# NVIDIAGameWorks/kaolin-wisp

Measured on NVIDIA B200. Metric: rays/sec (fwd+bwd) 1024^2 Lego NeRF HashGrid, higher is better.
Workload: dtype f16(tensor)+f32 accumulate

## Files before the change

### kaolin-wisp_b200/csrc/wb_shade_tc.cu

```cuda
#include "wb_common.cuh"
#include "wb_featx.cuh"
#include "wb_tc.cuh"
#include <math.h>

#define TC_ML 16
constexpr int TC_ROWS = 128;
constexpr int TC_GROUP = 256;
constexpr int TC_BWD_GROUPS = 2;
constexpr int TC_ISSUERS = 2;

struct WbTc {
    int nl_d, nl_c;
    int I[TC_ML], O[TC_ML], Kp[TC_ML], Np[TC_ML];
    int w_off[TC_ML], b_off[TC_ML];
    int has_bias;
    int ones_off;
    int src_w[TC_ML], src_b[TC_ML];
    int blob_bytes;
    int tile_off[TC_ML];
    int dy_off[2];
    int sub_off[2];
    int w_smem_off;
    int smem_bytes;
    int acc_col[TC_ML];
    int work_col[2];
    int tmem_cols;
    int feat_dim, pos_dim, view_dim, pos_mode, pos_freq, view_mode, view_freq;
    int fits2;
};

static int tc_round_up(int v, int m) { return (v + m - 1) / m * m; }

constexpr int TC_B3_GROUPS = 3;
struct TcB3Plan {
    int P, Q, R, E, GB, blob_off, ones_off, smem_bytes;
    int groups;
    int kind[8], acc_col[8], bias_col[8];
    int acc_begin, acc_end;
};

static bool tc_b3_plan(const WbTc& m, TcB3Plan* p)
{
    if (m.nl_d != 2 || m.nl_c != 3) return false;
    int maxw = 0, sumN = 0;
    for (int l = 0; l < 5; ++l) { maxw = max(maxw, max(m.Kp[l], m.Np[l])); sumN += m.Np[l]; }
    if (maxw > 128) return false;
    if (maxw > 64 && maxw != 128) return false;
    if (m.Kp[1] != maxw || m.Kp[3] != maxw || m.Kp[4] != maxw || m.Np[0] != maxw || m.Np[2] != maxw || m.Np[3] != maxw) return false;
    memset(p, 0, sizeof(*p));
    p->groups = (maxw <= 64 && sumN <= 512 - 3 * 64) ? 3 : 1;
    const int wc = p->groups == 3 ? 64 : 128;
    int col = p->groups * wc;
    p->acc_begin = col;
    for (int l = 0; l < 5; ++l) {
        p->kind[l] = p->groups == 3 ? 0 : (m.Kp[l] + 16 < m.Np[l] ? 2 : (m.Kp[l] >= 128 ? 1 : 0));
        p->acc_col[l] = col; col += p->kind[l] == 2 ? m.Kp[l] + 16 : m.Np[l];
        p->bias_col[l] = col; if (p->kind[l] == 1) col += 16;
    }
    p->acc_end = col;
    if (col > 512) return false;
    const int big = (maxw / 8 + 1) * 2048;
    const int small = (max(m.Np[1], m.Np[4]) / 8) * 2048;
    p->P = 0; p->Q = big; p->R = 2 * big; p->E = 3 * big; p->GB = 3 * big + small;
    p->blob_off = p->groups * p->GB;
    p->ones_off = p->blob_off + m.blob_bytes;
    int end = p->ones_off + 2 * 2048;
    const int window = (p->groups - 1) * p->GB + (p->groups == 3 ? p->R : p->E) + 16 * 2048;
    if (end < window) end = window;
    p->smem_bytes = end + 64;
    return p->smem_bytes + 6144 <= 227 * 1024;
}


static int tc_embed_dim(int mode, int freq) { return mode == 0 ? 0 : mode == 1 ? 3 : mode == 2 ? 6 * freq : 3 + 6 * freq; }

int wb_tc_make(const wb_nef_desc* d, bool backward, WbTc* m, bool tmem_a = false)
{
    WB_CHECK_ARG(d->dens_layers >= 1 && d->col_layers >= 1 && d->dens_layers + d->col_layers <= TC_ML, "unsupported decoder depth");
    WB_CHECK_ARG(d->dens_params && d->col_params, "null decoder parameters");
    memset(m, 0, sizeof(*m));
    m->nl_d = d->dens_layers; m->nl_c = d->col_layers;
    m->feat_dim = d->multiscale == 0 ? d->num_lods * d->feature_dim : d->feature_dim;
    m->pos_mode = d->pos_mode; m->pos_freq = d->pos_freq; m->view_mode = d->view_mode; m->view_freq = d->view_freq;
    m->pos_dim = tc_embed_dim(d->pos_mode, d->pos_freq); m->view_dim = tc_embed_dim(d->view_mode, d->view_freq);
    WB_CHECK_ARG(d->dens_dims[0] == m->feat_dim + m->pos_dim, "decoder_density input width != grid features + position embedding");
    const int dout = d->dens_dims[d->dens_layers];
    WB_CHECK_ARG(dout >= 2 && dout <= 16, "tensor-core path: decoder_density output must be 2..16 wide");
    WB_CHECK_ARG(d->col_dims[0] == dout - 1 + m->view_dim, "decoder_color input width != density feats - 1 + view embedding");
    WB_CHECK_ARG(d->col_dims[d->col_layers] == 3, "decoder_color output must be 3 wide");
    const int nl = m->nl_d + m->nl_c;
    int off = 0, srcd = 0, srcc = 0, maxw = 0;
    for (int l = 0; l < nl; ++l) {
        const bool dens = l < m->nl_d;
        const int I = dens ? d->dens_dims[l] : d->col_dims[l - m->nl_d];
        const int O = dens ? d->dens_dims[l + 1] : d->col_dims[l - m->nl_d + 1];
        WB_CHECK_ARG(I >= 1 && I <= 128 && O >= 1 && O <= 128, "tensor-core path: layer widths must be <= 128");
        m->I[l] = I; m->O[l] = O; m->Kp[l] = tc_round_up(I, 16); m->Np[l] = tc_round_up(O, 16);
        m->w_off[l] = off; off += m->Kp[l] * m->Np[l] * 2;
        m->b_off[l] = off; off += m->Np[l] * 32;
        int& src = dens ? srcd : srcc;
        m->src_w[l] = src; src += I * O;
        if (d->has_bias) { m->src_b[l] = src; src += O; } else m->src_b[l] = -1;
        maxw = max(maxw, max(m->Kp[l], m->Np[l]));
    }
    m->blob_bytes = tc_round_up(off, 16);
    m->has_bias = d->has_bias ? 1 : 0;
    int sub_bytes = 0;
    if (backward) {
        for (int l = 0; l < nl; ++l) { m->tile_off[l] = sub_bytes; sub_bytes += (m->Kp[l] / 8 + 1) * 2048; }
    } else {
        for (int l = 0; l < nl; ++l) m->tile_off[l] = 0;
        sub_bytes = (maxw / 8) * 2048;
    }
    const int groups = backward ? TC_BWD_GROUPS : 1;
    m->sub_off[0] = 0; m->sub_off[1] = sub_bytes;
    int p = groups * sub_bytes;
    if (backward) { m->dy_off[0] = p; p += (maxw / 8) * 2048; m->dy_off[1] = p; p += (maxw / 8) * 2048; }
    m->w_smem_off = p; p += m->blob_bytes;
    m->ones_off = p; p += 2 * 2048;
    if (backward) {
        const int need = m->sub_off[groups - 1] + m->tile_off[nl - 1] + 16 * 2048;
        if (p < need) p = need;
    }
    m->smem_bytes = p + 64;
    const bool smem2 = m->smem_bytes + (backward ? 5632 : 3584) <= 227 * 1024;
    int col = 0;
    for (int gi = 0; gi < groups; ++gi) { m->work_col[gi] = col; col += maxw; }
    if (tmem_a && !backward) { m->work_col[1] = col; col += maxw / 2; }
    if (backward) for (int l = 0; l < nl; ++l) { m->acc_col[l] = col; col += m->Np[l]; }
    m->fits2 = (smem2 && col <= 512) ? 1 : 0;
    if (!m->fits2) {
        TcB3Plan plan3;
        WB_CHECK_ARG(backward && tc_b3_plan(*m, &plan3),
                     !smem2 ? (backward ? "tensor-core path: decoder backward does not fit in shared memory (use precision 0)"
                                        : "tensor-core path: decoder does not fit in shared memory (use precision 0)")
                            : "tensor-core path: accumulators do not fit in TMEM (use precision 0)");
        col = 512;
    }
    int alloc = 32; while (alloc < col) alloc <<= 1;
    m->tmem_cols = alloc;
    return WB_OK;
}

static void tc_dfeat_shape(const wb_nef_desc* d, int* planes, int* width)
{
    *width = d->feature_dim;
    *planes = d->multiscale == 0 ? (d->lod_idx < d->num_lods ? d->lod_idx : d->num_lods) : 1;
    if (*planes < 0) *planes = 0;
}
static int64_t tc_align256(int64_t b) { return (b + 255) / 256 * 256; }

int64_t wb_tc_workspace_bytes(const wb_nef_desc* nef, int64_t R, int64_t S, int backward)
{
    WbTc m; if (wb_tc_make(nef, false, &m)) return -1;
    int planes, width; tc_dfeat_shape(nef, &planes, &width);
    int64_t b = tc_align256(R * m.Kp[m.nl_d] * 2);
    if (backward) b += tc_align256((int64_t)planes * S * width * 2);
    return b + 256;
}
int wb_tc_supported(const wb_nef_desc* nef, int backward)
{
    WbTc m; if (wb_tc_make(nef, false, &m)) return 0;
    if (backward && wb_tc_make(nef, true, &m)) return 0;
    return 1;
}
int64_t wb_tc_feat_bytes(const wb_nef_desc* nef, int64_t S)
{
    WbTc m; if (wb_tc_make(nef, true, &m) || wb_tc_make(nef, false, &m)) return -1;
    return (int64_t)m.Kp[0] * 2 * S + 256;
}

__global__ void wb_tc_pack_kernel(WbTc m, const float* __restrict__ dens, const float* __restrict__ col, uint8_t* __restrict__ blob)
{
    const int nl = m.nl_d + m.nl_c;
    for (int l = 0; l < nl; ++l) {
        const float* src = l < m.nl_d ? dens : col;
        const int I = m.I[l], O = m.O[l], Kp = m.Kp[l], Np = m.Np[l];
        __half* w = reinterpret_cast<__half*>(blob + m.w_off[l]);
        for (int e = blockIdx.x * blockDim.x + threadIdx.x; e < Kp * Np; e += gridDim.x * blockDim.x) {
            const int kc = e / (Np * 8), n = (e / 8) % Np, k = kc * 8 + (e & 7);
            w[e] = __float2half_rn((n < O && k < I) ? src[m.src_w[l] + n * I + k] : 0.0f);
        }
        __half* b = reinterpret_cast<__half*>(blob + m.b_off[l]);
        for (int e = blockIdx.x * blockDim.x + threadIdx.x; e < Np * 16; e += gridDim.x * blockDim.x) {
            const int kc = e / (Np * 8), n = (e / 8) % Np, k = kc * 8 + (e & 7);
            b[e] = __float2half_rn((k == 0 && n < O && m.src_b[l] >= 0) ? src[m.src_b[l] + n] : 0.0f);
// ... 708 lines not shown
                            if (dist >= o) { v0[j] += a; v1[j] += b; }
                        }
                    }
                }
                if (tail && valid) {
                    float2* t2 = reinterpret_cast<float2*>(tb);
#pragma unroll
                    for (int j = 0; j < 4; ++j) {
                        const uint32_t i0 = idx[j], i1 = idx[j + 4];
                        const bool nz0 = (v0[j] != 0.0f || v1[j] != 0.0f), nz1 = (v0[j + 4] != 0.0f || v1[j + 4] != 0.0f);
                        if (pair_ok && ((i0 ^ i1) == 1u)) {
                            if (nz0 || nz1) {
                                const float4 val = (i0 & 1u) ? make_float4(v0[j + 4], v1[j + 4], v0[j], v1[j]) : make_float4(v0[j], v1[j], v0[j + 4], v1[j + 4]);
                                atomicAdd(reinterpret_cast<float4*>(t2 + (i0 & ~1u)), val);
                            }
                        } else {
                            if (nz0) atomicAdd(t2 + i0, make_float2(v0[j], v1[j]));
                            if (nz1) atomicAdd(t2 + i1, make_float2(v0[j + 4], v1[j + 4]));
                        }
                    }
                }
            } else {
                for (int f = 0; f < Fr; ++f) {
                    float v[8];
#pragma unroll
                    for (int j = 0; j < 8; ++j) v[j] = gv[f] * cf[j];
                    for (int o = 1; o <= maxd; o <<= 1) {
#pragma unroll
                        for (int j = 0; j < 8; ++j) { const float a = __shfl_up_sync(0xffffffffu, v[j], o); if (dist >= o) v[j] += a; }
                    }
                    if (tail && valid) {
#pragma unroll
                        for (int j = 0; j < 8; ++j) if (v[j] != 0.0f) atomicAdd(tb + (int64_t)idx[j] * Fr + f, v[j]);
                    }
                }
            }
        }
    }
}

__global__ void __launch_bounds__(256)
wb_featx_scatter_kernel(WbGridX gx, TcIn in, const __half* __restrict__ dfeat, int width, const float* __restrict__ scale_p)
{
    const float inv_scale = 1.0f / __ldg(scale_p);
    const int lane = threadIdx.x & 31;
    const int64_t nwork = (in.S + 31) & ~(int64_t)31;
    for (int64_t s = (int64_t)blockIdx.x * blockDim.x + threadIdx.x; s < nwork; s += (int64_t)gridDim.x * blockDim.x) {
        const bool valid = s < in.S;
        float px = 0.0f, py = 0.0f, pz = 0.0f;
        if (valid) {
            const int64_t ray = __ldg(in.rec_ray + s);
            const float t = __ldg(in.rec_t + s);
            px = wb_addcmul(__ldg(in.origins + 3 * ray), __ldg(in.dirs + 3 * ray), t);
            py = wb_addcmul(__ldg(in.origins + 3 * ray + 1), __ldg(in.dirs + 3 * ray + 1), t);
            pz = wb_addcmul(__ldg(in.origins + 3 * ray + 2), __ldg(in.dirs + 3 * ray + 2), t);
        }
        auto grad = [&](int f) {
            return __half2float(dfeat[((int64_t)(f / width) * in.S + s) * width + (f % width)]) * inv_scale;
        };
        if (gx.kind != 1 || gx.C > 4) {
            if (valid) wb_featx_scatter(gx, px, py, pz, grad);
            continue;
        }
        const int C = gx.C;
        float gsum[3][4];
#pragma unroll
        for (int p = 0; p < 3; ++p)
#pragma unroll
            for (int c = 0; c < 4; ++c) gsum[p][c] = (gx.sum && valid && c < C) ? grad(p * C + c) : 0.0f;
        for (int l = 0; l < gx.nl; ++l) {
            const int size = gx.res[l] + 1; const int64_t hw = (int64_t)size * size;
#pragma unroll
            for (int p = 0; p < 3; ++p) {
                WbBilinear b = wb_tp_setup(px, py, pz, p, size);
                float v[4][4];
#pragma unroll
                for (int c = 0; c < 4; ++c) {
                    const float g = gx.sum ? gsum[p][c] : ((valid && c < C) ? grad((l * 3 + p) * C + c) : 0.0f);
                    v[0][c] = g * b.nw; v[1][c] = g * b.ne; v[2][c] = g * b.sw; v[3][c] = g * b.se;
                }
                const int key = valid ? b.o00 : -1 - lane;
                const int kprev = __shfl_up_sync(0xffffffffu, key, 1);
                const bool head = (lane == 0) || (kprev != key);
                const uint32_t heads = __ballot_sync(0xffffffffu, head);
                const int run_head = 31 - __clz(heads & (0xffffffffu >> (31 - lane)));
                const int dist = lane - run_head;
                const bool tail = (lane == 31) || ((heads >> (lane + 1)) & 1u);
                const int maxd = __reduce_max_sync(0xffffffffu, dist);
                for (int o = 1; o <= maxd; o <<= 1) {
#pragma unroll
                    for (int t4 = 0; t4 < 4; ++t4)
#pragma unroll
                        for (int c = 0; c < 4; ++c) {
                            const float a = __shfl_up_sync(0xffffffffu, v[t4][c], o);
                            if (dist >= o) v[t4][c] += a;
                        }
                }
                if (tail && valid && gx.chlast) {
                    float4* t4 = reinterpret_cast<float4*>(gx.gptr[l * 3 + p]);
                    auto nz = [](const float* q) { return q[0] != 0.0f || q[1] != 0.0f || q[2] != 0.0f || q[3] != 0.0f; };
                    if (nz(v[0])) atomicAdd(t4 + b.o00, make_float4(v[0][0], v[0][1], v[0][2], v[0][3]));
                    if (b.bx1 && nz(v[1])) atomicAdd(t4 + b.o01, make_float4(v[1][0], v[1][1], v[1][2], v[1][3]));
                    if (b.by1 && nz(v[2])) atomicAdd(t4 + b.o10, make_float4(v[2][0], v[2][1], v[2][2], v[2][3]));
                    if (b.bx1 && b.by1 && nz(v[3])) atomicAdd(t4 + b.o11, make_float4(v[3][0], v[3][1], v[3][2], v[3][3]));
                } else if (tail && valid) {
                    float* pl = gx.gptr[l * 3 + p];
#pragma unroll
                    for (int c = 0; c < 4; ++c) {
                        if (c >= C) break;
                        float* ch = pl + c * hw;
                        if (v[0][c] != 0.0f) atomicAdd(ch + b.o00, v[0][c]);
                        if (b.bx1 && v[1][c] != 0.0f) atomicAdd(ch + b.o01, v[1][c]);
                        if (b.by1 && v[2][c] != 0.0f) atomicAdd(ch + b.o10, v[2][c]);
                        if (b.bx1 && b.by1 && v[3][c] != 0.0f) atomicAdd(ch + b.o11, v[3][c]);
                    }
                }
            }
        }
    }
}

#include "wb_shade_tc_bwd3.cuh"

int wb_tc_decoder_bwd_ex(const wb_nef_desc* nef, const float* blob, const wb_rays* rays, const float* rec_t, const int32_t* rec_ray,
                         int64_t S, const float* g_shaded, const float* scale, const void* feat_saved, void* workspace,
                         float* grad_dens, float* grad_col, float* grad_table, int* fused_out, cudaStream_t st);
int wb_tc_decoder_bwd(const wb_nef_desc* nef, const float* blob, const wb_rays* rays, const float* rec_t, const int32_t* rec_ray,
                      int64_t S, const float* g_shaded, const float* scale, const void* feat_saved, void* workspace,
                      float* grad_dens, float* grad_col, cudaStream_t st)
{
    return wb_tc_decoder_bwd_ex(nef, blob, rays, rec_t, rec_ray, S, g_shaded, scale, feat_saved, workspace, grad_dens, grad_col, nullptr, nullptr, st);
}
int wb_tc_decoder_bwd_ex(const wb_nef_desc* nef, const float* blob, const wb_rays* rays, const float* rec_t, const int32_t* rec_ray,
                         int64_t S, const float* g_shaded, const float* scale, const void* feat_saved, void* workspace,
                         float* grad_dens, float* grad_col, float* grad_table, int* fused_out, cudaStream_t st)
{
    if (fused_out) *fused_out = 0;
    WbTc m; int rc = wb_tc_make(nef, true, &m); if (rc) return rc;
    WB_CHECK_ARG(scale != nullptr, "precision 1 needs the device loss-scale pointer");
    WB_CHECK_ARG(feat_saved != nullptr && workspace != nullptr, "precision 1 backward needs the saved features and the workspace");
    if (g_tc_skip_embed) g_tc_skip_embed = 0;
    else { rc = tc_launch_ray_embed(m, rays, workspace, st); if (rc) return rc; }
    int planes, width; tc_dfeat_shape(nef, &planes, &width);
    const int64_t R = rays->num_rays;
    __half* dfeat = reinterpret_cast<__half*>(reinterpret_cast<uint8_t*>(workspace) + tc_align256(R * m.Kp[m.nl_d] * 2));
    TcIn in = { rays->origins, rays->dirs, rec_t, rec_ray, S, reinterpret_cast<const uint4*>(workspace), nullptr, reinterpret_cast<const uint4*>(feat_saved),
                g_tc_s_begin, g_tc_s_end };
    const int64_t S_launch = (g_tc_s_end ? g_tc_s_end : S) - g_tc_s_begin;
    TcGrads G = { grad_dens, grad_col, scale, dfeat, planes, width };
    TcB3Plan plan;
    if (tc_b3_plan(m, &plan)) {
        WbGrid g; memset(&g, 0, sizeof(g));
        const bool fuse = grad_table != nullptr && nef->grid_kind == 0 && nef->feature_dim == 2 && nef->multiscale == 0 && planes <= 16 &&
                          plan.groups == 3;
        if (fuse) { rc = wb_make_grid(nef, &g); if (rc) return rc; }
        using Bwd3Kernel = decltype(&wb_mlp_bwd3_tc_kernel<false, 3>);
        static const Bwd3Kernel kerns3[3] = { wb_mlp_bwd3_tc_kernel<false, 1>, wb_mlp_bwd3_tc_kernel<false, 3>, wb_mlp_bwd3_tc_kernel<true, 3> };
        const int variant = plan.groups == 1 ? 0 : fuse ? 2 : 1;
        const Bwd3Kernel kern3 = kerns3[variant];
        static int64_t done3[3] = { -1, -1, -1 };
        if (done3[variant] != WB_ATTR_KEY(plan.smem_bytes)) {
            WB_CUDA(cudaFuncSetAttribute(kern3, cudaFuncAttributeMaxDynamicSharedMemorySize, plan.smem_bytes));
            done3[variant] = WB_ATTR_KEY(plan.smem_bytes);
        }
        const int64_t nctas3 = ((S_launch + TC_ROWS - 1) / TC_ROWS + plan.groups - 1) / plan.groups;
        int64_t grid3 = (int64_t)wb_num_sms(); if (grid3 > nctas3) grid3 = nctas3;
        kern3<<<(unsigned)grid3, plan.groups * TC_GROUP, plan.smem_bytes, st>>>(m, plan, reinterpret_cast<const uint8_t*>(blob), in,
                                                                          reinterpret_cast<const float4*>(g_shaded), G, g, grad_table);
        WB_LAUNCH_CHECK();
        if (fuse && fused_out) *fused_out = 1;
        return WB_OK;
    }
    WB_CHECK_ARG(m.fits2, "tensor-core path: decoder backward does not fit in shared memory (use precision 0)");
    {
        static int64_t done_for = -1;
        if (done_for != WB_ATTR_KEY(m.smem_bytes)) {
            WB_CUDA(cudaFuncSetAttribute(wb_mlp_bwd_tc_kernel, cudaFuncAttributeMaxDynamicSharedMemorySize, m.smem_bytes));
            done_for = WB_ATTR_KEY(m.smem_bytes);
        }
    }
    const int64_t nctas = ((S + TC_ROWS - 1) / TC_ROWS + TC_BWD_GROUPS - 1) / TC_BWD_GROUPS;
    int64_t grid = (int64_t)wb_num_sms(); if (grid > nctas) grid = nctas;
    wb_mlp_bwd_tc_kernel<<<(unsigned)grid, TC_BWD_GROUPS * TC_GROUP, m.smem_bytes, st>>>(m, reinterpret_cast<const uint8_t*>(blob), in,
                                                                           reinterpret_cast<const float4*>(g_shaded), G);
    WB_LAUNCH_CHECK();
    return WB_OK;
}
int wb_tc_table_scatter(const wb_nef_desc* nef, const wb_rays* rays, const float* rec_t, const int32_t* rec_ray, int64_t S,
                        const float* scale, void* workspace, float* grad_table, cudaStream_t st)
{
    WbGrid g; int rc = wb_make_grid(nef, &g); if (rc) return rc;
    WbGridX gx; rc = wb_make_gridx(nef, true, &gx); if (rc) return rc;
    WbTc m; rc = wb_tc_make(nef, true, &m); if (rc) return rc;
    WB_CHECK_ARG(scale != nullptr && workspace != nullptr && (grad_table != nullptr || gx.kind != 0), "null pointer");
    int planes, width; tc_dfeat_shape(nef, &planes, &width);
    const int64_t R = rays->num_rays;
    const __half* dfeat = reinterpret_cast<const __half*>(reinterpret_cast<const uint8_t*>(workspace) + tc_align256(R * m.Kp[m.nl_d] * 2));
    TcIn in = { rays->origins, rays->dirs, rec_t, rec_ray, S, nullptr, nullptr, nullptr, gx.kind != 0 ? 0 : g_tc_s_begin, gx.kind != 0 ? 0 : g_tc_s_end };
    const int64_t S_launch = gx.kind != 0 ? S : (g_tc_s_end ? g_tc_s_end : S) - g_tc_s_begin;
    if (gx.kind != 0) {
        int64_t bx = (S + 255) / 256; const int64_t cap = (int64_t)wb_num_sms() * 16; if (bx > cap) bx = cap;
        wb_featx_scatter_kernel<<<(unsigned)bx, 256, 0, st>>>(gx, in, dfeat, width, scale);
        WB_LAUNCH_CHECK();
        return WB_OK;
    }
    const int levels = g.multiscale == 0 ? planes : g.L;
    if (levels > 0) {
        const int lpb = max(1, min(levels, TC_SCATTER_LPB));
        int64_t bx = (S_launch + 255) / 256; const int64_t cap = (int64_t)wb_num_sms() * TC_SCATTER_CTAS; if (bx > cap) bx = cap;
        dim3 grid2((unsigned)bx, (unsigned)((levels + lpb - 1) / lpb));
        auto kern = g.F == 2 ? wb_table_scatter_kernel<2> : wb_table_scatter_kernel<0>;
        kern<<<grid2, 256, 0, st>>>(g, in, dfeat, planes, levels, lpb, scale, grad_table, g.F == 2);
        WB_LAUNCH_CHECK();
    }
    return WB_OK;
}

struct TcSide { cudaStream_t stream; cudaEvent_t ev[TC_WIDE_CHUNKS + 1]; bool ok; };
static TcSide* tc_side_stream()
{
    static TcSide side[64];
    int dev = 0; if (cudaGetDevice(&dev) != cudaSuccess || dev < 0 || dev >= 64) return nullptr;
    TcSide& s = side[dev];
    if (!s.ok) {
        if (cudaStreamCreateWithFlags(&s.stream, cudaStreamNonBlocking) != cudaSuccess) return nullptr;
        for (int i = 0; i <= TC_WIDE_CHUNKS; ++i) if (cudaEventCreateWithFlags(&s.ev[i], cudaEventDisableTiming) != cudaSuccess) return nullptr;
        s.ok = true;
    }
    return &s;
}

int wb_tc_shade_bwd(const wb_nef_desc* nef, const float* blob, const wb_rays* rays, const float* rec_t, const int32_t* rec_ray,
                    int64_t S, const float* g_shaded, const float* scale, const void* feat_saved, void* workspace,
                    float* grad_table, float* grad_dens, float* grad_col, cudaStream_t st)
{
    {
        WbTc m; TcB3Plan plan;
        TcSide* side = nullptr;
        if (S >= TC_WIDE_MIN_S && nef->grid_kind == 0 && grad_table && wb_tc_make(nef, true, &m) == WB_OK && !m.fits2 &&
            tc_b3_plan(m, &plan) && plan.groups == 1 && (side = tc_side_stream()) != nullptr) {
            const int64_t per = ((S + TC_WIDE_CHUNKS - 1) / TC_WIDE_CHUNKS + TC_ROWS - 1) / TC_ROWS * TC_ROWS;
            int rc = WB_OK, c = 0;
            for (int64_t s0 = 0; s0 < S && rc == WB_OK; s0 += per, ++c) {
                g_tc_s_begin = s0; g_tc_s_end = s0 + per < S ? s0 + per : S;
                if (c > 0) g_tc_skip_embed = 1;
                rc = wb_tc_decoder_bwd_ex(nef, blob, rays, rec_t, rec_ray, S, g_shaded, scale, feat_saved, workspace, grad_dens, grad_col, nullptr, nullptr, st);
                if (rc == WB_OK && (cudaEventRecord(side->ev[c], st) != cudaSuccess || cudaStreamWaitEvent(side->stream, side->ev[c], 0) != cudaSuccess)) rc = WB_ERR_CUDA;
                if (rc == WB_OK) rc = wb_tc_table_scatter(nef, rays, rec_t, rec_ray, S, scale, workspace, grad_table, side->stream);
            }
            g_tc_s_begin = 0; g_tc_s_end = 0;
            if (cudaEventRecord(side->ev[TC_WIDE_CHUNKS], side->stream) != cudaSuccess || cudaStreamWaitEvent(st, side->ev[TC_WIDE_CHUNKS], 0) != cudaSuccess) { if (rc == WB_OK) rc = WB_ERR_CUDA; }
            return rc;
        }
    }
    int fused = 0;
    int rc = wb_tc_decoder_bwd_ex(nef, blob, rays, rec_t, rec_ray, S, g_shaded, scale, feat_saved, workspace, grad_dens, grad_col, grad_table, &fused, st);
    if (rc || fused) return rc;
    return wb_tc_table_scatter(nef, rays, rec_t, rec_ray, S, scale, workspace, grad_table, st);
}
```

### kaolin-wisp_b200/csrc/wb_shade_tc_bwd3.cuh

```cuda
#pragma once

constexpr int TC_B3_ROUNDS = 11;

template <int NG>
__device__ __forceinline__ void tc_b3_build_table(const WbTc& m, const TcB3Plan& p, TcRec* tab, uint8_t* smem, uint32_t tmem)
{
    constexpr int WC = NG == 3 ? 64 : 128;
    const int e = threadIdx.x;
    if (e < TC_ROWS) {
        uint4 one; one.x = 0x00003C00u; one.y = 0; one.z = 0; one.w = 0;
        *reinterpret_cast<uint4*>(smem + p.ones_off + e * 16) = one;
        *reinterpret_cast<uint4*>(smem + p.ones_off + 2048 + e * 16) = make_uint4(0, 0, 0, 0);
    }
    if (e >= NG * TC_B3_ROUNDS * 3) return;
    const int ch = e % 3, rd = (e / 3) % TC_B3_ROUNDS, g = e / (3 * TC_B3_ROUNDS);
    const uint32_t base = tc_smem_u32(smem), gb = base + g * p.GB;
    const uint32_t bP = gb + p.P, bQ = gb + p.Q, bR = gb + p.R, bE = gb + p.E;
    const uint32_t wbase = base + p.blob_off;
    const uint32_t work = tmem + g * WC;
    const int  lay[TC_B3_ROUNDS] = { 0, 1, 2, 3, 4, 4, 3, 2, 0, 1, 0 };
    const bool fwd[TC_B3_ROUNDS] = { true, true, true, true, true, false, false, false, true, false, false };
    const uint32_t X[TC_B3_ROUNDS] = { bP, bQ, bR, bP, bQ, bQ, bP, bR, bR, bQ, bR };
    const uint32_t Y[TC_B3_ROUNDS] = { 0, 0, 0, 0, 0, bE, bQ, bP, 0, bE, bQ };
    const int l = lay[rd], Np = m.Np[l], Kp = m.Kp[l];
    uint64_t da = 0, db = 0; uint32_t id = 0, d = 0, nk = 0, acc = 0, aadv = 0, badv = 0;
    if (fwd[rd]) {
        if (ch == 0) {
            da = tc_desc(base + p.ones_off, 2048, 128); db = tc_desc(wbase + m.b_off[l], Np * 16, 128);
            id = tc_idesc(128, Np, 0, 0); d = work; nk = m.has_bias ? 1 : 0;
        } else if (ch == 1) {
            da = tc_desc(X[rd], 2048, 128); db = tc_desc(wbase + m.w_off[l], Np * 16, 128);
            id = tc_idesc(128, Np, 0, 0); d = work; nk = Kp / 16; acc = m.has_bias; aadv = 4096 >> 4; badv = (2 * Np * 16) >> 4;
        }
    } else {
        if (ch == 0 && p.kind[l] != 2) {
            da = tc_desc(X[rd], 128, 2048); db = tc_desc(Y[rd], 128, 2048);
            id = tc_idesc(128, Np, 1, 1); d = tmem + p.acc_col[l]; nk = 8; acc = 1; aadv = 256 >> 4; badv = 256 >> 4;
        } else if (ch == 0) {
            da = tc_desc(Y[rd], 128, 2048); db = tc_desc(X[rd], 128, 2048);
            id = tc_idesc(128, Kp + 16, 1, 1); d = tmem + p.acc_col[l]; nk = 8; acc = 1; aadv = 256 >> 4; badv = 256 >> 4;
        } else if (ch == 1 && p.kind[l] == 1) {
            da = tc_desc(Y[rd], 128, 2048); db = tc_desc(X[rd] + (uint32_t)(Kp / 8) * 2048u, 128, 2048);
            id = tc_idesc(128, 16, 1, 1); d = tmem + p.bias_col[l]; nk = m.has_bias ? 8 : 0; acc = 1; aadv = 256 >> 4; badv = 256 >> 4;
        } else if (ch == 2) {
            da = tc_desc(Y[rd], 2048, 128); db = tc_desc(wbase + m.w_off[l], 128, Np * 16);
            id = tc_idesc(128, Kp, 0, 1); d = work; nk = Np / 16; aadv = 4096 >> 4; badv = 256 >> 4;
        }
    }
    TcRec r = { (uint32_t)da, (uint32_t)(da >> 32), (uint32_t)db, (uint32_t)(db >> 32), id, d, nk | (acc << 8), aadv | (badv << 16) };
    tab[(g * TC_B3_ROUNDS + rd) * 3 + ch] = r;
}

__device__ __forceinline__ void tc_b3_round(TcCtx& c, const TcRec* r3)
{
    uint4 qa0 = make_uint4(0, 0, 0, 0), qa1 = qa0, qb0 = qa0, qb1 = qa0;
    if (c.wig == 0) {
        const uint4* pa = reinterpret_cast<const uint4*>(r3); const uint4* pb = reinterpret_cast<const uint4*>(r3 + 1);
        qa0 = pa[0]; qa1 = pa[1]; qb0 = pb[0]; qb1 = pb[1];
    } else if (c.wig == 1) {
        const uint4* pa = reinterpret_cast<const uint4*>(r3 + 2);
        qa0 = pa[0]; qa1 = pa[1];
    }
    tc_fence_smem_async();
    tc_fence_before();
    tc_group_sync(c.g + 1, TC_GROUP);
    if (c.wig < TC_ISSUERS) {
        if (tc_elect_one()) {
            tc_fence_after();
            if (((qa1.z | qb1.z) & 0xffu) != 0) { tc_issue_rec(qa0, qa1); tc_issue_rec(qb0, qb1); tc_commit(c.bar); }
            else tc_mbar_arrive(c.bar);
        }
        __syncwarp();
    }
    tc_mbar_wait(c.bar, c.phase);
    c.phase ^= 1u;
    tc_fence_after();
}

__device__ __forceinline__ void tc_b3_relu_to_tile(const TcCtx& c, uint32_t trow, int Np, uint8_t* dst)
{
    for (int c0 = c.h * 32; c0 < Np; c0 += 64) {
        for (int cc = c0; cc < min(c0 + 32, Np); cc += 16) {
            float v[16]; tc_ld16(trow + cc, v);
#pragma unroll
            for (int q = 0; q < 2; ++q) {
                uint4 o;
                o.x = tc_pack2_relu(v[q * 8], v[q * 8 + 1]); o.y = tc_pack2_relu(v[q * 8 + 2], v[q * 8 + 3]);
                o.z = tc_pack2_relu(v[q * 8 + 4], v[q * 8 + 5]); o.w = tc_pack2_relu(v[q * 8 + 6], v[q * 8 + 7]);
                *reinterpret_cast<uint4*>(dst + ((cc >> 3) + q) * 2048 + c.r * 16) = o;
            }
        }
    }
}
__device__ __forceinline__ void tc_b3_mask_in_place(const TcCtx& c, uint32_t trow, int Kp, uint8_t* tile)
{
    for (int c0 = c.h * 32; c0 < Kp; c0 += 64) {
        for (int cc = c0; cc < min(c0 + 32, Kp); cc += 16) {
            float v[16]; tc_ld16(trow + cc, v);
#pragma unroll
            for (int q = 0; q < 2; ++q) {
                uint4* slot = reinterpret_cast<uint4*>(tile + ((cc >> 3) + q) * 2048 + c.r * 16);
                const uint4 a = *slot;
                const __half2 z2 = __float2half2_rn(0.0f);
                uint4 o;
                o.x = tc_pack2(v[q * 8], v[q * 8 + 1]) & __hgt2_mask(*reinterpret_cast<const __half2*>(&a.x), z2);
                o.y = tc_pack2(v[q * 8 + 2], v[q * 8 + 3]) & __hgt2_mask(*reinterpret_cast<const __half2*>(&a.y), z2);
                o.z = tc_pack2(v[q * 8 + 4], v[q * 8 + 5]) & __hgt2_mask(*reinterpret_cast<const __half2*>(&a.z), z2);
                o.w = tc_pack2(v[q * 8 + 6], v[q * 8 + 7]) & __hgt2_mask(*reinterpret_cast<const __half2*>(&a.w), z2);
                *slot = o;
            }
        }
    }
}
__device__ __forceinline__ void tc_b3_one_slab(uint8_t* tile, int slab, int r)
{
    uint4 one; one.x = 0x00003C00u; one.y = 0; one.z = 0; one.w = 0;
    *reinterpret_cast<uint4*>(tile + slab * 2048 + r * 16) = one;
}

__device__ __forceinline__ void tc_scatter_level_f2(const WbGrid& g, int l, float px, float py, float pz, bool valid, float s0, float s1,
                                                    float inv_scale, int lane, float* __restrict__ gtable)
{
    float* tb = gtable + g.begin[l] * 2;
    const bool pair_ok = (reinterpret_cast<uintptr_t>(tb) & 15u) == 0;
    uint32_t idx[8]; float cf[8]; uint64_t key = ~0ull - (uint64_t)lane;
    if (valid) {
        int ix, iy, iz; float wx, wy, wz, jx, jy, jz;
        wb_cell(px, g.hres[l], g.hi[l], ix, wx, jx); wb_cell(py, g.hres[l], g.hi[l], iy, wy, jy); wb_cell(pz, g.hres[l], g.hi[l], iz, wz, jz);
        key = (uint64_t)ix | ((uint64_t)iy << 20) | ((uint64_t)iz << 40);
        const float xy00 = jx * jy, xy01 = jx * wy, xy10 = wx * jy, xy11 = wx * wy;
        cf[0] = xy00 * jz; cf[1] = xy00 * wz; cf[2] = xy01 * jz; cf[3] = xy01 * wz;
        cf[4] = xy10 * jz; cf[5] = xy10 * wz; cf[6] = xy11 * jz; cf[7] = xy11 * wz;
        wb_corner_indices(g, l, ix, iy, iz, idx);
    } else {
#pragma unroll
        for (int j = 0; j < 8; ++j) { idx[j] = 0; cf[j] = 0.0f; }
    }
    const uint64_t kprev = __shfl_up_sync(0xffffffffu, key, 1);
    const bool head = (lane == 0) || (kprev != key);
    const uint32_t heads = __ballot_sync(0xffffffffu, head);
    const int run_head = 31 - __clz(heads & (0xffffffffu >> (31 - lane)));
    const int dist = lane - run_head;
    const bool tail = (lane == 31) || ((heads >> (lane + 1)) & 1u);
    const int maxd = __reduce_max_sync(0xffffffffu, dist);
    float v0[8], v1[8];
    if (maxd > 0) {
        __half2 h[8];
#pragma unroll
        for (int j = 0; j < 8; ++j) h[j] = __floats2half2_rn(s0 * cf[j], s1 * cf[j]);
        for (int o = 1; o <= maxd; o <<= 1) {
#pragma unroll
            for (int j = 0; j < 8; ++j) {
                const __half2 a = __shfl_up_sync(0xffffffffu, h[j], o);
                if (dist >= o) h[j] = __hadd2(h[j], a);
            }
        }
#pragma unroll
        for (int j = 0; j < 8; ++j) { const float2 f = __half22float2(h[j]); v0[j] = f.x * inv_scale; v1[j] = f.y * inv_scale; }
    } else {
        const float g0 = s0 * inv_scale, g1 = s1 * inv_scale;
#pragma unroll
        for (int j = 0; j < 8; ++j) { v0[j] = g0 * cf[j]; v1[j] = g1 * cf[j]; }
    }
    if (tail && valid) {
        float2* t2 = reinterpret_cast<float2*>(tb);
#pragma unroll
        for (int j = 0; j < 4; ++j) {
            const uint32_t i0 = idx[j], i1 = idx[j + 4];
            const bool nz0 = (v0[j] != 0.0f || v1[j] != 0.0f), nz1 = (v0[j + 4] != 0.0f || v1[j + 4] != 0.0f);
            if (pair_ok && ((i0 ^ i1) == 1u)) {
                if (nz0 || nz1) {
                    const float4 val = (i0 & 1u) ? make_float4(v0[j + 4], v1[j + 4], v0[j], v1[j]) : make_float4(v0[j], v1[j], v0[j + 4], v1[j + 4]);
                    atomicAdd(reinterpret_cast<float4*>(t2 + (i0 & ~1u)), val);
                }
            } else {
                if (nz0) atomicAdd(t2 + i0, make_float2(v0[j], v1[j]));
                if (nz1) atomicAdd(t2 + i1, make_float2(v0[j + 4], v1[j + 4]));
            }
        }
    }
}

template <bool FUSE, int NG = TC_B3_GROUPS>
__global__ void __launch_bounds__(NG * TC_GROUP, 1)
wb_mlp_bwd3_tc_kernel(WbTc m, TcB3Plan p, const uint8_t* __restrict__ blob, TcIn in, const float4* __restrict__ g_shaded, TcGrads G, WbGrid g, float* __restrict__ gtable)
{
    constexpr int WC = NG == 3 ? 64 : 128;
    extern __shared__ __align__(1024) uint8_t smem[];
    __shared__ __align__(8) uint64_t bars[NG + 1];
    __shared__ uint32_t tmem_s;
    __shared__ TcRec tab[NG * TC_B3_ROUNDS * 3];
    if (threadIdx.x == 0) {
        for (int i = 0; i < NG; ++i) tc_mbar_init(&bars[i], TC_ISSUERS);
        tc_mbar_init(&bars[NG], 1); tc_mbar_init_fence();
        tc_mbar_expect_tx(&bars[NG], (uint32_t)m.blob_bytes);
        tc_bulk_g2s(smem + p.blob_off, blob, (uint32_t)m.blob_bytes, &bars[NG]);
    }
    if (threadIdx.x < 32) tc_tmem_alloc(&tmem_s, 512u);
    tc_fence_before();
    __syncthreads();
    tc_fence_after();
    tc_b3_build_table<NG>(m, p, tab, smem, tmem_s);
    TcCtx c; tc_ctx_init(c, smem, bars, nullptr, tmem_s, 1);
    uint8_t* gbase = smem + c.g * p.GB;
    uint8_t* bP = gbase + p.P; uint8_t* bQ = gbase + p.Q; uint8_t* bR = gbase + p.R; uint8_t* bE = gbase + p.E;
    const TcRec* rec = tab + c.g * TC_B3_ROUNDS * 3;
    const int maxslab = (p.Q - p.P) / 2048 - 1;
    if (c.h == 0) { tc_b3_one_slab(bP, maxslab, c.r); tc_b3_one_slab(bQ, maxslab, c.r); }
    if (threadIdx.x < 128) {
        const uint32_t tr = c.tmem + ((uint32_t)c.laneq << 16);
        for (int cc = p.acc_begin; cc < p.acc_end; cc += 16) tc_st16_zero(tr + cc);
    }
    tc_fence_before();
    __syncthreads();
    tc_fence_after();
    tc_mbar_wait(&bars[NG], 0);
    const float scale = __ldg(G.scale), inv_scale = 1.0f / scale;
    const int nch0 = m.Kp[0] / 8, nchc = m.Kp[2] / 8;
    const int64_t s_end = in.s_end ? in.s_end : in.S;
    const int64_t tile0 = in.s_begin / TC_ROWS, ntiles = (s_end + TC_ROWS - 1) / TC_ROWS;
    const uint32_t trow = c.tmem + ((uint32_t)c.laneq << 16) + (uint32_t)(c.g * WC);
    const float z8[8] = { 0, 0, 0, 0, 0, 0, 0, 0 };
    const int lane_ = threadIdx.x & 31;
    for (int64_t tile = tile0 + (int64_t)blockIdx.x * NG + c.g; tile < ntiles; tile += (int64_t)gridDim.x * NG) {
        int64_t s = tile * TC_ROWS + c.r;
        const bool valid = s < s_end;
        if (!valid) s = s_end - 1;
        const int64_t ray = __ldg(in.rec_ray + s);
        for (int ch = c.h; ch < nch0; ch += 2)
            *reinterpret_cast<uint4*>(bP + ch * 2048 + c.r * 16) = __ldg(in.x0_saved + (int64_t)ch * in.S + s);
        if (c.h == 0) tc_b3_one_slab(bP, nch0, c.r);
        tc_b3_round(c, rec + 0 * 3);
        tc_b3_relu_to_tile(c, trow, m.Np[0], bQ);
        tc_b3_round(c, rec + 1 * 3);
        float df0;
        {
            float df[16];
            tc_ld16(trow, df);
            df0 = df[0];
            const int nd = m.O[1] - 1;
            const uint4* re = in.ray_embed + ray * nchc;
            uint4 q = __ldg(re + c.h);
            __half* hq = reinterpret_cast<__half*>(&q);
#pragma unroll
            for (int j = 0; j < 8; ++j) {
                const float dv = c.h == 0 ? df[(j + 1) & 15] : df[(j + 9) & 15];
                if (8 * c.h + j < nd) hq[j] = __float2half_rn(dv);
            }
            *reinterpret_cast<uint4*>(bR + c.h * 2048 + c.r * 16) = q;
            for (int ch = 2 + c.h; ch < nchc; ch += 2) *reinterpret_cast<uint4*>(bR + ch * 2048 + c.r * 16) = __ldg(re + ch);
            if (c.h == 0) tc_b3_one_slab(bR, nchc, c.r);
        }
        tc_b3_round(c, rec + 2 * 3);
        tc_b3_relu_to_tile(c, trow, m.Np[2], bP);
        tc_b3_round(c, rec + 3 * 3);
        tc_b3_relu_to_tile(c, trow, m.Np[3], bQ);
        tc_b3_round(c, rec + 4 * 3);
        const float4 go = valid ? __ldg(g_shaded + s) : make_float4(0, 0, 0, 0);
        {
            float v[16]; tc_ld16(trow, v);
            if (c.h == 0) {
                const float r = 1.0f / (1.0f + expf(-v[0])), gg = 1.0f / (1.0f + expf(-v[1])), b = 1.0f / (1.0f + expf(-v[2]));
                float dy[8] = { go.x * r * (1.0f - r) * scale, go.y * gg * (1.0f - gg) * scale, go.z * b * (1.0f - b) * scale, 0, 0, 0, 0, 0 };
                tile_store8(bE, c.r, 0, dy);
            }
            for (int sl = 1 + c.h; sl < m.Np[4] / 8; sl += 2) tile_store8(bE, c.r, sl, z8);
        }
        tc_b3_round(c, rec + 5 * 3);
        tc_b3_mask_in_place(c, trow, m.Kp[4], bQ);
        tc_b3_round(c, rec + 6 * 3);
        tc_b3_mask_in_place(c, trow, m.Kp[3], bP);
        tc_b3_round(c, rec + 7 * 3);
        {
            float v[16]; tc_ld16(trow, v);
            const int dout = m.O[1];
            float gdf[16];
            gdf[0] = (df0 > 0.0f) ? go.w * scale : 0.0f;
#pragma unroll
            for (int j = 1; j < 16; ++j) gdf[j] = (j < dout) ? v[j - 1] : 0.0f;
            if (c.h == 0) tile_store8(bE, c.r, 0, gdf); else tile_store8(bE, c.r, 1, gdf + 8);
            for (int sl = 2 + c.h; sl < m.Np[1] / 8; sl += 2) tile_store8(bE, c.r, sl, z8);
            for (int ch = c.h; ch < nch0; ch += 2)
                *reinterpret_cast<uint4*>(bR + ch * 2048 + c.r * 16) = __ldg(in.x0_saved + (int64_t)ch * in.S + s);
            if (c.h == 0) tc_b3_one_slab(bR, nch0, c.r);
        }
        tc_b3_round(c, rec + 8 * 3);
        tc_b3_relu_to_tile(c, trow, m.Np[0], bQ);
        tc_b3_round(c, rec + 9 * 3);
        tc_b3_mask_in_place(c, trow, m.Kp[1], bQ);
        float px = 0.0f, py = 0.0f, pz = 0.0f;
        if (FUSE) {
            const float t = __ldg(in.rec_t + s);
            px = wb_addcmul(__ldg(in.origins + 3 * ray), __ldg(in.dirs + 3 * ray), t);
            py = wb_addcmul(__ldg(in.origins + 3 * ray + 1), __ldg(in.dirs + 3 * ray + 1), t);
            pz = wb_addcmul(__ldg(in.origins + 3 * ray + 2), __ldg(in.dirs + 3 * ray + 2), t);
        }
        tc_b3_round(c, rec + 10 * 3);
        if (FUSE) {
            float v[16]; tc_ld16(trow + c.h * 16, v);
#pragma unroll
            for (int q = 0; q < 8; ++q) {
                const int l = c.h * 8 + q;
                if (l < G.planes) tc_scatter_level_f2(g, l, px, py, pz, valid, v[2 * q], v[2 * q + 1], inv_scale, lane_, gtable);
            }
        } else {
            const int W = G.width, nfe = G.planes * W;
            for (int f0 = c.h * 16; f0 < nfe; f0 += 32) {
                float v[16]; tc_ld16(trow + f0, v);
                if (!valid) continue;
                if (W == 2) {
#pragma unroll
                    for (int qq = 0; qq < 8; ++qq) {
                        const int pl = (f0 >> 1) + qq;
                        if (pl < G.planes) reinterpret_cast<__half2*>(G.dfeat)[(int64_t)pl * in.S + s] = __floats2half2_rn(v[2 * qq], v[2 * qq + 1]);
                    }
                } else {
#pragma unroll
                    for (int jj = 0; jj < 16; ++jj) {
                        const int fe = f0 + jj;
                        if (fe < nfe) G.dfeat[((int64_t)(fe / W) * in.S + s) * W + (fe % W)] = __float2half_rn(v[jj]);
                    }
                }
            }
        }
    }
    tc_fence_before();
    __syncthreads();
    tc_fence_after();
    if (threadIdx.x < 128) {
        const int row = threadIdx.x;
        const uint32_t tr = c.tmem + ((uint32_t)c.laneq << 16);
        for (int l = 0; l < 5; ++l) {
            float* gbase2 = l < m.nl_d ? G.gdens : G.gcol;
            const int I = m.I[l], O = m.O[l];
            const int wrow0 = row & ~31;
            if (p.kind[l] == 2) {
                if (wrow0 >= m.Np[l]) continue;
                for (int cc = 0; cc < m.Kp[l] + 16; cc += 16) {
                    float v[16]; tc_ld16(tr + p.acc_col[l] + cc, v);
                    if (row >= O) continue;
#pragma unroll
                    for (int j = 0; j < 16; ++j) {
                        const int i = cc + j;
                        const float val = v[j] * inv_scale;
                        if (i < I) { if (val != 0.0f) atomicAdd(gbase2 + m.src_w[l] + row * I + i, val); }
                        else if (i == m.Kp[l] && m.src_b[l] >= 0) atomicAdd(gbase2 + m.src_b[l] + row, val);
                    }
                }
                continue;
            }
            if (p.kind[l] == 1 && m.src_b[l] >= 0 && wrow0 < m.Np[l]) {
                float v[16]; tc_ld16(tr + p.bias_col[l], v);
                if (row < O) atomicAdd(gbase2 + m.src_b[l] + row, v[0] * inv_scale);
            }
            if (wrow0 > m.Kp[l]) continue;
            for (int cc = 0; cc < m.Np[l]; cc += 16) {
                float v[16]; tc_ld16(tr + p.acc_col[l] + cc, v);
#pragma unroll
                for (int j = 0; j < 16; ++j) {
                    const int o = cc + j;
                    if (o >= O) continue;
                    const float val = v[j] * inv_scale;
                    if (row < I) { if (val != 0.0f) atomicAdd(gbase2 + m.src_w[l] + o * I + row, val); }
                    else if (p.kind[l] == 0 && row == m.Kp[l] && m.src_b[l] >= 0) atomicAdd(gbase2 + m.src_b[l] + o, val);
                }
            }
        }
    }
    tc_fence_before();
    __syncthreads();
    if (threadIdx.x < 32) tc_tmem_dealloc(c.tmem, 512u);
}
```

Baseline: 94.84 million.

## Offload fused hash-grid gradient scatter to dedicated warps via TMEM handoff

Adds a warp-specialized group of scatter threads to the fused backward MLP kernel. The last MMA round now writes feature gradients into a dedicated TMEM hand-off region per group, guarded by full/empty mbarriers, so the MLP warps can move on to the next tile while separate warps do the atomic hash-grid scatter. This aims to overlap the atomic-heavy scatter with tensor-core work. It costs extra TMEM columns and 128 more threads per CTA, and the issuer now blocks until the scatter warps have drained the previous tile's buffer.

```diff
diff --git a/kaolin-wisp_b200/csrc/wb_shade_tc.cu b/kaolin-wisp_b200/csrc/wb_shade_tc.cu
--- a/kaolin-wisp_b200/csrc/wb_shade_tc.cu
+++ b/kaolin-wisp_b200/csrc/wb_shade_tc.cu
@@ -32,6 +32,8 @@
 static int tc_round_up(int v, int m) { return (v + m - 1) / m * m; }
 
 constexpr int TC_B3_GROUPS = 3;
+constexpr int TC_B3_SCATTER = 128;
+constexpr int TC_B3_HAND = 32;
 struct TcB3Plan {
     int P, Q, R, E, GB, blob_off, ones_off, smem_bytes;
     int groups;
@@ -1046,7 +1048,7 @@
     if (tc_b3_plan(m, &plan)) {
         WbGrid g; memset(&g, 0, sizeof(g));
         const bool fuse = grad_table != nullptr && nef->grid_kind == 0 && nef->feature_dim == 2 && nef->multiscale == 0 && planes <= 16 &&
-                          plan.groups == 3;
+                          plan.groups == 3 && m.Kp[0] <= TC_B3_HAND && plan.acc_end + TC_B3_GROUPS * TC_B3_HAND <= 512;
         if (fuse) { rc = wb_make_grid(nef, &g); if (rc) return rc; }
         using Bwd3Kernel = decltype(&wb_mlp_bwd3_tc_kernel<false, 3>);
         static const Bwd3Kernel kerns3[3] = { wb_mlp_bwd3_tc_kernel<false, 1>, wb_mlp_bwd3_tc_kernel<false, 3>, wb_mlp_bwd3_tc_kernel<true, 3> };
@@ -1059,7 +1061,7 @@
         }
         const int64_t nctas3 = ((S_launch + TC_ROWS - 1) / TC_ROWS + plan.groups - 1) / plan.groups;
         int64_t grid3 = (int64_t)wb_num_sms(); if (grid3 > nctas3) grid3 = nctas3;
-        kern3<<<(unsigned)grid3, plan.groups * TC_GROUP, plan.smem_bytes, st>>>(m, plan, reinterpret_cast<const uint8_t*>(blob), in,
+        kern3<<<(unsigned)grid3, plan.groups * TC_GROUP + (fuse ? TC_B3_SCATTER : 0), plan.smem_bytes, st>>>(m, plan, reinterpret_cast<const uint8_t*>(blob), in,
                                                                           reinterpret_cast<const float4*>(g_shaded), G, g, grad_table);
         WB_LAUNCH_CHECK();
         if (fuse && fused_out) *fused_out = 1;
diff --git a/kaolin-wisp_b200/csrc/wb_shade_tc_bwd3.cuh b/kaolin-wisp_b200/csrc/wb_shade_tc_bwd3.cuh
--- a/kaolin-wisp_b200/csrc/wb_shade_tc_bwd3.cuh
+++ b/kaolin-wisp_b200/csrc/wb_shade_tc_bwd3.cuh
@@ -2,7 +2,16 @@
 
 constexpr int TC_B3_ROUNDS = 11;
 
-template <int NG>
+#ifdef WB_TC_TIMING
+__device__ long long g_tc_hand[4][TC_TS_N];
+#define TC_B3_HAND_TS(n, row) do { if (blockIdx.x == 0 && (n) < TC_TS_N) g_tc_hand[(row)][(n)++] = clock64(); } while (0)
+extern "C" int wb_tc_timing_dump5(long long* out)
+{ return (int)cudaMemcpyFromSymbol(out, g_tc_hand, sizeof(long long) * 4 * TC_TS_N); }
+#else
+#define TC_B3_HAND_TS(n, row) do { } while (0)
+#endif
+
+template <int NG, bool FUSE>
 __device__ __forceinline__ void tc_b3_build_table(const WbTc& m, const TcB3Plan& p, TcRec* tab, uint8_t* smem, uint32_t tmem)
 {
     constexpr int WC = NG == 3 ? 64 : 128;
@@ -44,14 +53,14 @@
             id = tc_idesc(128, 16, 1, 1); d = tmem + p.bias_col[l]; nk = m.has_bias ? 8 : 0; acc = 1; aadv = 256 >> 4; badv = 256 >> 4;
         } else if (ch == 2) {
             da = tc_desc(Y[rd], 2048, 128); db = tc_desc(wbase + m.w_off[l], 128, Np * 16);
-            id = tc_idesc(128, Kp, 0, 1); d = work; nk = Np / 16; aadv = 4096 >> 4; badv = 256 >> 4;
+            id = tc_idesc(128, Kp, 0, 1); d = (FUSE && rd == 10) ? tmem + p.acc_end + g * TC_B3_HAND : work; nk = Np / 16; aadv = 4096 >> 4; badv = 256 >> 4;
         }
     }
     TcRec r = { (uint32_t)da, (uint32_t)(da >> 32), (uint32_t)db, (uint32_t)(db >> 32), id, d, nk | (acc << 8), aadv | (badv << 16) };
     tab[(g * TC_B3_ROUNDS + rd) * 3 + ch] = r;
 }
 
-__device__ __forceinline__ void tc_b3_round(TcCtx& c, const TcRec* r3)
+__device__ __forceinline__ void tc_b3_round(TcCtx& c, const TcRec* r3, uint64_t* full = nullptr, uint64_t* empty = nullptr, uint32_t empty_parity = 0)
 {
     uint4 qa0 = make_uint4(0, 0, 0, 0), qa1 = qa0, qb0 = qa0, qb1 = qa0;
     if (c.wig == 0) {
@@ -67,8 +76,15 @@
     if (c.wig < TC_ISSUERS) {
         if (tc_elect_one()) {
             tc_fence_after();
-            if (((qa1.z | qb1.z) & 0xffu) != 0) { tc_issue_rec(qa0, qa1); tc_issue_rec(qb0, qb1); tc_commit(c.bar); }
-            else tc_mbar_arrive(c.bar);
+            const bool hand = full != nullptr && c.wig == 1;
+            if (hand) {
+                TC_B3_HAND_TS(c.tsn, c.g);
+                tc_mbar_wait(empty, empty_parity);
+                TC_B3_HAND_TS(c.tsn, c.g);
+                tc_fence_after();
+            }
+            if (((qa1.z | qb1.z) & 0xffu) != 0) { tc_issue_rec(qa0, qa1); tc_issue_rec(qb0, qb1); tc_commit(c.bar); if (hand) tc_commit(full); }
+            else { tc_mbar_arrive(c.bar); if (hand) tc_mbar_arrive(full); }
         }
         __syncwarp();
     }
@@ -181,17 +197,70 @@
     }
 }
 
+template <int NG> __device__ __forceinline__ int64_t tc_b3_first(int64_t tile0, int g) { return tile0 + (int64_t)blockIdx.x * NG + g; }
+template <int NG> __device__ __forceinline__ int64_t tc_b3_next(int64_t tile) { return tile + (int64_t)gridDim.x * NG; }
+__device__ __forceinline__ int64_t tc_b3_ntiles(int64_t s_end) { return (s_end + TC_ROWS - 1) / TC_ROWS; }
+
+template <int NG>
+__device__ __forceinline__ void tc_b3_scatter(const TcIn& in, const TcGrads& G, const WbGrid& g, float* __restrict__ gtable, uint32_t hand,
+                                              uint64_t* full, uint64_t* empty)
+{
+    const int r = threadIdx.x - NG * TC_GROUP, lane = threadIdx.x & 31;
+    const uint32_t trow = hand + ((uint32_t)(r & ~31) << 16);
+    const float inv_scale = 1.0f / __ldg(G.scale);
+    const int64_t s_end = in.s_end ? in.s_end : in.S;
+    const int64_t tile0 = in.s_begin / TC_ROWS, ntiles = tc_b3_ntiles(s_end);
+#ifdef WB_TC_TIMING
+    int tsn = 0;
+#endif
+    uint32_t parity = 0;
+    for (int64_t t0 = tc_b3_first<NG>(tile0, 0); t0 < ntiles; t0 = tc_b3_next<NG>(t0), parity ^= 1u) {
+        for (int gi = 0; gi < NG && t0 + gi < ntiles; ++gi) {
+            int64_t s = (t0 + gi) * TC_ROWS + r;
+            const bool valid = s < s_end;
+            if (!valid) s = s_end - 1;
+            const int64_t ray = __ldg(in.rec_ray + s);
+            const float t = __ldg(in.rec_t + s);
+            const float px = wb_addcmul(__ldg(in.origins + 3 * ray), __ldg(in.dirs + 3 * ray), t);
+            const float py = wb_addcmul(__ldg(in.origins + 3 * ray + 1), __ldg(in.dirs + 3 * ray + 1), t);
+            const float pz = wb_addcmul(__ldg(in.origins + 3 * ray + 2), __ldg(in.dirs + 3 * ray + 2), t);
+            if (r == 0) TC_B3_HAND_TS(tsn, 3);
+            tc_mbar_wait(full + gi, parity);
+            if (r == 0) TC_B3_HAND_TS(tsn, 3);
+            tc_fence_after();
+            float v[16];
+#pragma unroll
+            for (int half = 0; half < 2; ++half) {
+                tc_ld16(trow + gi * TC_B3_HAND + half * 16, v);
+                if (half == 1) {
+                    tc_fence_before();
+                    __syncwarp();
+                    if (lane == 0) tc_mbar_arrive(empty + gi);
+                }
+#pragma unroll
+                for (int q = 0; q < 8; ++q) {
+                    const int l = half * 8 + q;
+                    if (l < G.planes) tc_scatter_level_f2(g, l, px, py, pz, valid, v[2 * q], v[2 * q + 1], inv_scale, lane, gtable);
+                }
+            }
+        }
+    }
+}
+
 template <bool FUSE, int NG = TC_B3_GROUPS>
-__global__ void __launch_bounds__(NG * TC_GROUP, 1)
+__global__ void __launch_bounds__(NG * TC_GROUP + (FUSE ? TC_B3_SCATTER : 0), 1)
 wb_mlp_bwd3_tc_kernel(WbTc m, TcB3Plan p, const uint8_t* __restrict__ blob, TcIn in, const float4* __restrict__ g_shaded, TcGrads G, WbGrid g, float* __restrict__ gtable)
 {
     constexpr int WC = NG == 3 ? 64 : 128;
     extern __shared__ __align__(1024) uint8_t smem[];
-    __shared__ __align__(8) uint64_t bars[NG + 1];
+    __shared__ __align__(8) uint64_t bars[NG + 1 + (FUSE ? 2 * NG : 0)];
     __shared__ uint32_t tmem_s;
     __shared__ TcRec tab[NG * TC_B3_ROUNDS * 3];
+    uint64_t* const full = bars + NG + 1;
+    uint64_t* const empty = full + NG;
     if (threadIdx.x == 0) {
         for (int i = 0; i < NG; ++i) tc_mbar_init(&bars[i], TC_ISSUERS);
+        if (FUSE) for (int i = 0; i < NG; ++i) { tc_mbar_init(&full[i], 1); tc_mbar_init(&empty[i], TC_B3_SCATTER / 32); }
         tc_mbar_init(&bars[NG], 1); tc_mbar_init_fence();
         tc_mbar_expect_tx(&bars[NG], (uint32_t)m.blob_bytes);
         tc_bulk_g2s(smem + p.blob_off, blob, (uint32_t)m.blob_bytes, &bars[NG]);
@@ -200,7 +269,17 @@
     tc_fence_before();
     __syncthreads();
     tc_fence_after();
-    tc_b3_build_table<NG>(m, p, tab, smem, tmem_s);
+    tc_b3_build_table<NG, FUSE>(m, p, tab, smem, tmem_s);
+    if (FUSE && threadIdx.x >= NG * TC_GROUP) {
+        tc_fence_before();
+        __syncthreads();
+        tc_fence_after();
+        tc_b3_scatter<NG>(in, G, g, gtable, tmem_s + p.acc_end, full, empty);
+        tc_fence_before();
+        __syncthreads();
+        __syncthreads();
+        return;
+    }
     TcCtx c; tc_ctx_init(c, smem, bars, nullptr, tmem_s, 1);
     uint8_t* gbase = smem + c.g * p.GB;
     uint8_t* bP = gbase + p.P; uint8_t* bQ = gbase + p.Q; uint8_t* bR = gbase + p.R; uint8_t* bE = gbase + p.E;
@@ -218,11 +297,11 @@
     const float scale = __ldg(G.scale), inv_scale = 1.0f / scale;
     const int nch0 = m.Kp[0] / 8, nchc = m.Kp[2] / 8;
     const int64_t s_end = in.s_end ? in.s_end : in.S;
-    const int64_t tile0 = in.s_begin / TC_ROWS, ntiles = (s_end + TC_ROWS - 1) / TC_ROWS;
+    const int64_t tile0 = in.s_begin / TC_ROWS, ntiles = tc_b3_ntiles(s_end);
     const uint32_t trow = c.tmem + ((uint32_t)c.laneq << 16) + (uint32_t)(c.g * WC);
     const float z8[8] = { 0, 0, 0, 0, 0, 0, 0, 0 };
-    const int lane_ = threadIdx.x & 31;
-    for (int64_t tile = tile0 + (int64_t)blockIdx.x * NG + c.g; tile < ntiles; tile += (int64_t)gridDim.x * NG) {
+    uint32_t empty_parity = 1;
+    for (int64_t tile = tc_b3_first<NG>(tile0, c.g); tile < ntiles; tile = tc_b3_next<NG>(tile)) {
         int64_t s = tile * TC_ROWS + c.r;
         const bool valid = s < s_end;
         if (!valid) s = s_end - 1;
@@ -288,21 +367,9 @@
         tc_b3_relu_to_tile(c, trow, m.Np[0], bQ);
         tc_b3_round(c, rec + 9 * 3);
         tc_b3_mask_in_place(c, trow, m.Kp[1], bQ);
-        float px = 0.0f, py = 0.0f, pz = 0.0f;
+        tc_b3_round(c, rec + 10 * 3, FUSE ? full + c.g : nullptr, FUSE ? empty + c.g : nullptr, empty_parity);
         if (FUSE) {
-            const float t = __ldg(in.rec_t + s);
-            px = wb_addcmul(__ldg(in.origins + 3 * ray), __ldg(in.dirs + 3 * ray), t);
-            py = wb_addcmul(__ldg(in.origins + 3 * ray + 1), __ldg(in.dirs + 3 * ray + 1), t);
-            pz = wb_addcmul(__ldg(in.origins + 3 * ray + 2), __ldg(in.dirs + 3 * ray + 2), t);
-        }
-        tc_b3_round(c, rec + 10 * 3);
-        if (FUSE) {
-            float v[16]; tc_ld16(trow + c.h * 16, v);
-#pragma unroll
-            for (int q = 0; q < 8; ++q) {
-                const int l = c.h * 8 + q;
-                if (l < G.planes) tc_scatter_level_f2(g, l, px, py, pz, valid, v[2 * q], v[2 * q + 1], inv_scale, lane_, gtable);
-            }
+            empty_parity ^= 1u;
         } else {
             const int W = G.width, nfe = G.planes * W;
             for (int f0 = c.h * 16; f0 < nfe; f0 += 32) {
```

Result: slower. 53.05 million, median of 6 (-44.1%).
